# 14chanwa/remotesensingProject

Hardware: AMD Instinct MI355X
Metric: Mpixel*disparity-hypotheses/s (higher is better)
Workload: dtype f32

## Files before the change

remotesensingproject_amd/build.py:

```python
from __future__ import annotations

import os
import re
import subprocess
import sys

HERE = os.path.dirname(os.path.abspath(__file__))
CSRC = os.path.join(HERE, "csrc")
OBJ = os.path.join(CSRC, "build")
SO = os.path.join(CSRC, "librslf_hip.so")
INCLUDE = os.path.join(os.path.dirname(HERE), "include")
COMMON = ["rslf_internal.hpp", "rslf_plan.hpp", "rslf_scratch.hpp", "rslf_device.hpp", os.path.join(INCLUDE, "rslf_hip.h")]
UNITS = {
    "rslf_core.hip": ["k0_pack.hpp"],
    "rslf_pile.hip": ["k1_edge.hpp", "k_compact.hpp", "k2_scan.hpp", "k2_reg.hpp", "k2_stream.hpp", "k3_median.hpp"],
    "rslf_chip_a.hip": ["k2_scan.hpp", "k2_chip.hpp"],
    "rslf_chip_b.hip": ["k2_scan.hpp", "k2_chip.hpp"],
    "rslf_chip_c.hip": ["k2_scan.hpp", "k2_chip.hpp"],
    "rslf_sweep.hip": ["k3_median.hpp", "k4_propagate.hpp", "k_compact.hpp", "k2_scan.hpp", "k7_line_conf.hpp"],
    "rslf_f2c.hip": ["k5_f2c.hpp"],
    "rslf_render.hip": ["k6_render.hpp", "rslf_plan_render.hpp"],
    "rslf_multi.hip": [],
    "rslf_multi_sweep.hip": [],
}
SOURCES = list(UNITS)

HIPCC_FLAGS = [
    "--offload-arch=gfx950",
    "-O3",
    "-std=c++17",
    "-fPIC",
    "-ffp-contract=off",
    "-fno-fast-math",
    "-fno-slp-vectorize",
]


def _hipcc() -> str:
    for c in (os.environ.get("HIPCC"), "/opt/rocm/bin/hipcc", "hipcc"):
        if c and (os.path.isabs(c) and os.path.exists(c) or not os.path.isabs(c)):
            return c
    raise RuntimeError("hipcc not found")


def _deps(unit: str) -> list[str]:
# ... 114 lines not shown
```

remotesensingproject_amd/csrc/k2_reg.hpp:

```cpp
#pragma once

#include "k2_scan.hpp"

namespace rslf {

#ifndef RSLF_REG_GB104
#define RSLF_REG_GB104 8
#endif
constexpr int gather_batch(int c) { return c == 1 ? 8 : 4; }
constexpr int kPadSlack = 16;

template <int SPAD, int C, bool PK, bool KONLY>
__device__ __forceinline__ void mean_shift_pass(const float (&R)[PK ? 1 : C][PK ? 1 : SPAD], const f2 (&R2)[PK ? C : 1][PK ? SPAD / 2 : 1],
                                                int S, float kq, const float (&rbar)[C], float (&A)[C], float& B)
{
    static_assert(!KONLY || (C == 1 && !PK), "the K-only pass is written for the scalar one-channel blocks");
    if constexpr (PK) {
        f2 rb2[C];
        const f2 kq2 = {kq, kq};
#pragma unroll
        for (int c = 0; c < C; c++)
            rb2[c] = f2{rbar[c], rbar[c]};
        constexpr int kBlk = (C == 1) ? 8 : 4;
#pragma unroll
        for (int s0 = 0; s0 < SPAD; s0 += kBlk) {
            if (!(s0 < SPAD - kPadSlack || s0 < S))
                continue;
            if constexpr (C == 1) {
                f2 P[4], K[4];
                const f2 r4[4] = {R2[0][s0 / 2], R2[0][s0 / 2 + 1], R2[0][s0 / 2 + 2], R2[0][s0 / 2 + 3]};
                mean_shift_pk_octet(r4, rb2[0], kq2, P, K);
#pragma unroll
                for (int j = 0; j < 4; j++) {
                    A[0] = A[0] + P[j].x;
                    B = B + K[j].x;
// ... 41 lines not shown
                        else
                            mean_shift_group1(R[0][s0 + j], rbar[0], kq, A[0], B);
                    }
            }
        }
    } else {
#pragma unroll
        for (int s = 0; s < SPAD; s++) {
            if (!(s < SPAD - kPadSlack || s < S))
                continue;
            float q[C];
#pragma unroll
            for (int c = 0; c < C; c++) {
                const float delta = R[c][s] - rbar[c];
                const float tq = kq * delta;
                q[c] = tq * delta;
            }
            float qs = q[0];
            if (C == 3) {
                qs = q[0] + q[C - 1];
                qs = qs + q[C > 1 ? 1 : 0];
            }
            const float K = kernel_weight(qs);
#pragma unroll
            for (int c = 0; c < C; c++) {
                const float pr = R[c][s] * K;
                A[c] = A[c] + pr;
            }
            B = B + K;
        }
    }
}

template <int SPAD, int C, bool BORDER, bool UNIFORM_D, bool PK, int GB = 0, class BestT = Best<C>, bool LANE_D = false,
          bool TRIM = false>
__device__ __forceinline__ void scan_reg_body(const ScanArgs& a, int v, int u, int d0, int d1, BestT& best,
                                              float* __restrict__ otab, int dlane = 0, int dstep = 1)
{
    static_assert(!LANE_D || !UNIFORM_D, "hypotheses in the lanes: every lane has its own view offsets");
    constexpr int kGatherBatch = GB > 0 ? GB : (C == 1 && !PK && SPAD == 104 && RSLF_REG_GB104 == 13) ? 13 : gather_batch(C);
    static_assert(SPAD % kGatherBatch == 0 && (!PK || kGatherBatch % 2 == 0), "whole batches, whole pairs");
    static_assert(SPAD % 8 == 0, "slot counts are multiples of 8");
    const VolView& vol = a.vol;
    const float* epi = vol.row(v, 0);
    const float uf = (float)u;
    const int Um1 = vol.U - 1;
    const unsigned Um1_bits = __float_as_uint((float)Um1);
    const int S = vol.S;
    const int lane = threadIdx.x & 63;
    const long long o = (long long)v * vol.U + u;
    const float dmin = a.dmin_vu ? a.dmin_vu[o] : a.dmin;
    const float dmax = a.dmax_vu ? a.dmax_vu[o] : a.dmax;
    const float range = dmax - dmin;
    const float denom = (float)(a.dim_d - 1);
    const float kq = (C == 1) ? a.k.k1 : a.k.inv_h2;
    const float slope = a.k.slope;
    const int stride_s = (int)vol.stride_s;
    float centre[C];
#pragma unroll
    for (int c = 0; c < C; c++)
        centre[c] = epi[(long long)a.s_hat * vol.stride_s + u * C + c];

#pragma unroll 1
    for (int dk = d0; dk < d1; dk += (LANE_D ? dstep : 1)) {
        const int d = LANE_D ? min(dk + dlane, d1 - 1) : dk;
        const float Dd = hypothesis(dmin, range, denom, d);
        float R[PK ? 1 : C][PK ? 1 : SPAD];
        f2 R2[PK ? C : 1][PK ? SPAD / 2 : 1];
        int card = BORDER ? 0 : S;
        float Ss0 = (float)a.s_hat;
        asm volatile("" : "+v"(Ss0));
        int rowoff = 0;
        asm volatile("" : "+s"(rowoff));
        if (UNIFORM_D) {
#pragma unroll
            for (int s0 = 0; s0 < SPAD; s0 += 64) {
                const int s = s0 + lane;
                float off = (float)(a.s_hat - s) * Dd;
                off = off * slope;
                if (SPAD % 64 == 0 || s < SPAD)
                    otab[s] = off;
            }
            __builtin_amdgcn_wave_barrier();
        }
#pragma unroll
        for (int g = 0; g < SPAD / kGatherBatch; g++) {
            float tt[kGatherBatch], e0[C][kGatherBatch], e1[C][kGatherBatch];
            bool ok[kGatherBatch];
#pragma unroll
            for (int j = 0; j < kGatherBatch; j++) {
                const int s = g * kGatherBatch + j;
                tt[j] = 0.0f;
                ok[j] = false;
#pragma unroll
                for (int c = 0; c < C; c++) {
                    e0[c][j] = kSentinel;
                    e1[c][j] = 0.0f;
                }
                if (s < SPAD - kPadSlack || s < S) {
                    float x;
                    if (UNIFORM_D) {
                        x = otab[s];
                    } else {
                        x = (Ss0 - (float)s) * Dd;
                        x = x * slope;
                    }
                    x = x + uf;
                    tt[j] = lerp_weight(x);
                    int i0 = floor_to_int(x);
                    ok[j] = true;
                    if (BORDER) {
                        ok[j] = __float_as_uint(x) <= Um1_bits;
                        i0 = ok[j] ? i0 : 0;
                    }
                    const unsigned byteoff = (unsigned)(i0 * C + rowoff) << 2;
                    const float* p = (const float*)((const char*)epi + byteoff);
#pragma unroll
                    for (int c = 0; c < C; c++) {
                        e0[c][j] = p[c];
                        e1[c][j] = p[C + c];
                    }
                }
                rowoff += stride_s;
            }
#pragma unroll
            for (int j = 0; j < kGatherBatch; j++) {
                const int s = g * kGatherBatch + j;
                const float omt = 1.0f - tt[j];
#pragma unroll
                for (int c = 0; c < C; c++) {
                    const float m0 = omt * e0[c][j];
                    const float m1 = tt[j] * e1[c][j];
                    const float r = m0 + m1;
                    float val;
                    if (BORDER)
                        val = ok[j] ? r : kSentinel;
                    else
                        val = (s < SPAD - kPadSlack || s < S) ? r : kSentinel;
                    if constexpr (PK) {
                        if (s & 1)
                            R2[c][s >> 1].y = val;
                        else
                            R2[c][s >> 1].x = val;
                    } else {
                        R[c][s] = val;
                    }
                }
                if (BORDER)
                    card += ok[j] ? 1 : 0;
            }
            {
                const int b = g * kGatherBatch;
#pragma unroll
                for (int c = 0; c < C; c++) {
                    if constexpr (PK) {
                        asm volatile("" : "+v"(R2[c][b / 2]), "+v"(R2[c][b / 2 + 1]));
                        if (kGatherBatch == 8)
                            asm volatile("" : "+v"(R2[c][b / 2 + 2]), "+v"(R2[c][b / 2 + 3]));
                        static_assert(!PK || kGatherBatch == 4 || kGatherBatch == 8, "pair pinning is written for 4 and 8");
                    } else if (kGatherBatch != 4 && kGatherBatch != 8) {
#pragma unroll
                        for (int j = 0; j < kGatherBatch; j++)
                            asm volatile("" : "+v"(R[c][b + j]));
                    } else {
                        asm volatile("" : "+v"(R[c][b + 0]), "+v"(R[c][b + 1]), "+v"(R[c][b + 2]), "+v"(R[c][b + 3]));
                        if (kGatherBatch == 8)
                            asm volatile("" : "+v"(R[c][b + kGatherBatch - 4]), "+v"(R[c][b + kGatherBatch - 3]),
                                              "+v"(R[c][b + kGatherBatch - 2]), "+v"(R[c][b + kGatherBatch - 1]));
                    }
                }
                if (BORDER)
                    asm volatile("" : "+s"(rowoff), "+v"(Ss0), "+v"(card));
                else
                    asm volatile("" : "+s"(rowoff), "+v"(Ss0));
            }
        }

        float rbar[C];
#pragma unroll
        for (int c = 0; c < C; c++)
            rbar[c] = centre[c];
        float B = 0.0f;
// ... 102 lines not shown
};

constexpr int scan_reg_waves(int spad, int c)
{
    const int regs = ((c * spad + (c == 1 ? 64 : 96) + 7) / 8) * 8;
    const int w = 512 / regs;
    if (c == 1 && spad > 104 && spad <= 144) return 3;
    if (c == 1 && spad >= 80 && spad <= 88) return 4;
    if (c == 3 && spad >= 32 && spad <= 40) return 3;
    if (c == 1 && (spad == 48 || spad == 40)) return 5;
    if (c == 3 && spad == 24) return 4;
    if (c == 1 && spad == 16) return 7;
    return w > 8 ? 8 : (w < 1 ? 1 : w);
}

#ifndef RSLF_REG_BEST_LDS
#define RSLF_REG_BEST_LDS 1
#endif
constexpr bool scan_reg_best_in_lds(int spad, int c)
{
    if (!RSLF_REG_BEST_LDS)
        return false;
    if (c == 1)
        return spad == 16 || spad == 40 || spad == 48 || (spad >= 80 && spad <= 88) || (spad >= 104 && spad <= 144);
    return spad == 24 || spad == 40;
}

constexpr bool scan_reg_packed_math(int spad, int c) { return scan_reg_waves(spad, c) == 1; }

constexpr bool scan_reg_trim(int spad, int c)
{
    return c == 1 && !scan_reg_packed_math(spad, c) && spad != 48 && !(spad >= 80 && spad <= 88) && !(spad > 112 && spad <= 144);
}
template <int SPAD, int C>
using ScanRegRbarFix = std::conditional_t<scan_reg_trim(SPAD, C), LastPassRbar<C>, NoRbarFix>;

template <int SPAD, int C, class BestT>
__device__ __forceinline__ void scan_reg_rows(const ScanArgs& a, int v, int u, int d0, int d1, BestT& best, float* otab)
{
    constexpr bool PK = scan_reg_packed_math(SPAD, C);
    if (a.dmin_vu) {
        scan_reg_body<SPAD, C, true, false, PK, 0, BestT, false, scan_reg_trim(SPAD, C)>(a, v, u, d0, d1, best, otab);
        return;
    }
    const float max_ds = (float)max(a.s_hat, a.vol.S - 1 - a.s_hat);
    const float range = a.dmax - a.dmin, denom = (float)(a.dim_d - 1);
    const float uf = (float)u, Um1 = (float)(a.vol.U - 1);
    auto interior = [&](int d) -> bool {
        const float reach = max_ds * fabsf(hypothesis(a.dmin, range, denom, d)) * fabsf(a.k.slope) + 2.0f;
        return __all((uf - reach >= 0.0f) && (uf + reach <= Um1));
    };
    int d = d0;
    while (d < d1) {
        const bool in = interior(d);
        int e = d + 1;
        while (e < d1 && interior(e) == in)
            e++;
        if (in)
            scan_reg_body<SPAD, C, false, true, PK, 0, BestT, false, scan_reg_trim(SPAD, C)>(a, v, u, d, e, best, otab);
        else
            scan_reg_body<SPAD, C, true, true, PK, 0, BestT, false, scan_reg_trim(SPAD, C)>(a, v, u, d, e, best, otab);
        d = e;
    }
}

template <int SPAD, int C>
__global__ __launch_bounds__(64 * kScanWaves) __attribute__((amdgpu_waves_per_eu(scan_reg_waves(SPAD, C), scan_reg_waves(SPAD, C))))
void k2_scan_reg(ScanArgs a)
{
    __shared__ float s_otab[kScanWaves][SPAD];
    float* otab = s_otab[__builtin_amdgcn_readfirstlane(threadIdx.x >> 6)];
    constexpr bool kEpiDyn = false;
    float* const epi_lds = nullptr;
    const int epi_stride = 0;
    using Fix = ScanRegRbarFix<SPAD, C>;
    if constexpr (scan_reg_best_in_lds(SPAD, C)) {
        __shared__ float s_best[kScanWaves][BestLds<C>::kFloats];
        BestLds<C> running(s_best[__builtin_amdgcn_readfirstlane(threadIdx.x >> 6)]);
        RSLF_SCAN_ROW_TILE_FIX((running.init(), scan_reg_rows<SPAD, C>(a, v, u, d0, d1, running, otab), running.load(best)), Fix{})
    } else {
        RSLF_SCAN_ROW_TILE_FIX((scan_reg_rows<SPAD, C>(a, v, u, d0, d1, best, otab)), Fix{})
    }
}

#ifndef RSLF_PACKED_LONG_GB
#define RSLF_PACKED_LONG_GB 4
#endif
constexpr bool packed_long_unit(int spad, int c) { return c == 1 && spad >= 80 && spad <= 128 && spad % RSLF_PACKED_LONG_GB == 0; }
constexpr int packed_waves(int spad, int c) { return packed_long_unit(spad, c) ? 2 : scan_reg_waves(spad + 24, c); }
constexpr int packed_gather_batch(int spad, int c) { return packed_long_unit(spad, c) ? spad / RSLF_PACKED_LONG_GB : 0; }

template <int SPAD, int C>
__global__ __launch_bounds__(64 * kScanWaves) __attribute__((amdgpu_waves_per_eu(packed_waves(SPAD, C), packed_waves(SPAD, C))))
void k2_scan_reg_packed(ScanArgs a)
{
    constexpr bool kEpiDyn = false;
    float* const epi_lds = nullptr;
    const int epi_stride = 0;
    RSLF_SCAN_PACKED_LOOP((scan_reg_body<SPAD, C, true, false, packed_waves(SPAD, C) == 1, packed_gather_batch(SPAD, C)>(a, v, u, d0, d1, best, nullptr)))
}

#ifndef RSLF_PX_ROWLIKE
#define RSLF_PX_ROWLIKE 1
// ... 39 lines not shown
```

remotesensingproject_amd/csrc/k2_scan.hpp:

```cpp
#pragma once

#include <type_traits>

#include "rslf_device.hpp"

namespace rslf {

constexpr int kScanWaves = 4;
#ifndef RSLF_XCD_ROW_INTERLEAVE
#define RSLF_XCD_ROW_INTERLEAVE 1
#endif

struct ScanArgs {
    VolView vol;
    const int* list;
    const int* count;
    const float* dmin_vu;
    const float* dmax_vu;
    float dmin, dmax;
    int dim_d, s_hat;
    ScanConsts k;
    float* Ce;
    uint8_t* Ce_mask;
    float* Cd;
    float* depth;
    float* rbar;
    int32_t* idx;
    float* score;
    int tile_w;
    int tiles_per_row;
    int logical_blocks;
    int per_xcd;
    int groups;
    struct Partial* partial;
    int* ticket;
    int v0;
    int packed;
    const int* packed_n;
    int packed_adapt;
    int stream_park;
    int stream_wave_floats;
    float stream_frac_max;
    int px_waves;
    const int* rowbase;
    int row_min;
};

struct Partial {
    float score, D;
    int d;
    float rbar[3];
    double sum;
};

template <int C>
struct Best {
    float score;
    int d;
    float D;
    float rbar[C];
    double sum;
    __device__ __forceinline__ void init()
    {
        score = -1.0f;
        d = 0;
        D = 0.0f;
#pragma unroll
        for (int c = 0; c < C; c++)
            rbar[c] = 0.0f;
        sum = 0.0;
    }
    __device__ __forceinline__ void offer(float sc, int dd, float Dd, const float (&rb)[C])
    {
        sum += (double)sc;
        if (sc > score) {
            score = sc;
            d = dd;
            D = Dd;
// ... 540 lines not shown
```

remotesensingproject_amd/csrc/rslf_core.hip:

```cpp
#include "rslf_internal.hpp"

#include <algorithm>
#include <cmath>

#include "k0_pack.hpp"

using namespace rslf;


namespace rslf {

char* last_error_buffer()
{
    static thread_local char g_err[512] = "";
    return g_err;
}

static std::atomic<int> g_inject[kInjectSites];

bool inject_hit(InjectSite site)
{
    std::atomic<int>& c = g_inject[site];
    int v = c.load(std::memory_order_relaxed);
    while (v > 0)
// ... 182 lines not shown
        (void)hipEventDestroy(ctx->ev0);
    if (ctx->ev1)
        (void)hipEventDestroy(ctx->ev1);
    delete ctx;
    return RSLF_OK;
}
RSLF_API_CATCH

extern "C" int rslf_ctx_set_stream(rslf_ctx* ctx, void* hip_stream) RSLF_API_TRY
{
    if (!ctx)
        return fail(RSLF_ERR_INVALID_ARG, "ctx is NULL");
    ctx->stream = (hipStream_t)hip_stream;
    return RSLF_OK;
}
RSLF_API_CATCH

extern "C" int rslf_ctx_set_debug(rslf_ctx* ctx, const char* key, int value) RSLF_API_TRY
{
    if (!ctx || !key)
        return fail(RSLF_ERR_INVALID_ARG, "ctx/key is NULL");
    if (strcmp(key, "force_scan") == 0 && value >= 0 && value <= 2)
        ctx->force_scan = value;
    else if (strcmp(key, "force_groups") == 0 && value >= 0 && value <= 64)
        ctx->force_groups = value;
    else if (strcmp(key, "force_packed") == 0 && value >= -1 && value <= 1)
        ctx->force_packed = value;
    else if (strcmp(key, "px") == 0 && value >= -1 && value <= 1)
        ctx->px_mode = value;
    else if (strcmp(key, "stream_share") == 0 && value >= 0 && value <= 2)
        ctx->stream_share = value;
    else if (strcmp(key, "row_split") == 0 && value >= 0 && value <= 65536)
        ctx->row_split = value;
    else if (strcmp(key, "claim_skip") == 0 && (value == 0 || value == 1))
        ctx->claim_skip = value;
    else if (strcmp(key, "time_all") == 0 && (value == 0 || value == 1)) {
        ctx->time_all = value;
        ctx->ev_used = 0;
    } else if (strcmp(key, "stream_groups") == 0 && value >= 0 && value <= 64)
        ctx->stream_groups = value;
    else if (strcmp(key, "stream_lds_kib") == 0 && value >= 16 && value <= 152) {
        ctx->stream_lds_bytes = (size_t)value << 10;
    } else if (strcmp(key, "staging_kib") == 0 && value >= 0 && value <= 262144)
        ctx->staging_kib = value;
    else
        return fail(RSLF_ERR_INVALID_ARG, "rslf_ctx_set_debug: unknown key or value out of range: %s = %d", key, value);
    return RSLF_OK;
}
RSLF_API_CATCH

extern "C" int rslf_ctx_synchronize(rslf_ctx* ctx) RSLF_API_TRY
{
    if (!ctx)
        return fail(RSLF_ERR_INVALID_ARG, "ctx is NULL");
    HIP_TRY(hipSetDevice(ctx->device));
    HIP_TRY(hipStreamSynchronize(ctx->stream));
    return RSLF_OK;
}
RSLF_API_CATCH


extern "C" int rslf_volume_create(rslf_ctx* ctx, int V, int S, int U, int C, rslf_volume** out) RSLF_API_TRY
{
    if (!ctx || !out)
        return fail(RSLF_ERR_INVALID_ARG, "ctx/out is NULL");
    *out = nullptr;
// ... 474 lines not shown
```

remotesensingproject_amd/csrc/rslf_device.hpp:

```cpp
#pragma once

#include <hip/hip_runtime.h>
#include <stdint.h>

namespace rslf {

constexpr int kWave = 64;
constexpr float kSentinel = 1.0e30f;

struct VolView {
    const float* base;
    int V, S, U, C;
    int pitch;
    long long stride_s;
    long long stride_v;
    __device__ __forceinline__ const float* row(int v, int s) const
    {
        return base + (long long)v * stride_v + (long long)s * stride_s;
    }
};

struct ScanConsts {
    float slope;
    float inv_h2;
    float k1;
    float raw_thr;
    int   n_iter;
    int   interp;
};

struct EdgeConsts {
    int   filter_size;
    int   cut_shadows;
    float shadow_level;
    float edge_thr;
};

__device__ __forceinline__ float norm1(float x)
{
    return (float)((double)fabsf(x) * 1.73205080757);
}
__device__ __forceinline__ float norm3(float x, float y, float z)
{
    double s = (double)x * (double)x;
    s += (double)y * (double)y;
    s += (double)z * (double)z;
    return (float)sqrt(s);
}

__device__ __forceinline__ float kernel_weight(float q)
{
    float k;
    asm("v_sub_f32_e64 %0, 1.0, %1 clamp" : "=v"(k) : "v"(q));
    return k;
}

__device__ __forceinline__ float lerp_weight(float x)
{
    return __builtin_amdgcn_fractf(x);
}
__device__ __forceinline__ int floor_to_int(float x)
{
    int i;
    asm("v_cvt_flr_i32_f32_e32 %0, %1" : "=v"(i) : "v"(x));
    return i;
}

typedef float f2 __attribute__((ext_vector_type(2)));

__device__ __forceinline__ f2 kernel_weight_pk(f2 q)
{
    f2 k;
    const f2 one = {1.0f, 1.0f};
    asm("v_pk_add_f32 %0, %1, %2 neg_lo:[0,1] neg_hi:[0,1] clamp" : "=v"(k) : "v"(one), "v"(q));
    return k;
}

__device__ __forceinline__ void mean_shift_pk_octet(const f2 (&r)[4], f2 rb, f2 kq, f2 (&P)[4], f2 (&K)[4])
{
    const f2 one = {1.0f, 1.0f};
    f2 t0, t1, t2, t3;
    asm("v_pk_add_f32 %[k0], %[r0], %[rb] neg_lo:[0,1] neg_hi:[0,1]\n\t"
        "v_pk_add_f32 %[k1], %[r1], %[rb] neg_lo:[0,1] neg_hi:[0,1]\n\t"
        "v_pk_add_f32 %[k2], %[r2], %[rb] neg_lo:[0,1] neg_hi:[0,1]\n\t"
        "v_pk_add_f32 %[k3], %[r3], %[rb] neg_lo:[0,1] neg_hi:[0,1]\n\t"
        "v_pk_mul_f32 %[t0], %[kq], %[k0]\n\t"
        "v_pk_mul_f32 %[t1], %[kq], %[k1]\n\t"
        "v_pk_mul_f32 %[t2], %[kq], %[k2]\n\t"
        "v_pk_mul_f32 %[t3], %[kq], %[k3]\n\t"
        "v_pk_mul_f32 %[k0], %[k0], %[t0]\n\t"
        "v_pk_mul_f32 %[k1], %[k1], %[t1]\n\t"
        "v_pk_mul_f32 %[k2], %[k2], %[t2]\n\t"
        "v_pk_mul_f32 %[k3], %[k3], %[t3]\n\t"
        "v_pk_add_f32 %[k0], %[one], %[k0] neg_lo:[0,1] neg_hi:[0,1] clamp\n\t"
        "v_pk_add_f32 %[k1], %[one], %[k1] neg_lo:[0,1] neg_hi:[0,1] clamp\n\t"
        "v_pk_add_f32 %[k2], %[one], %[k2] neg_lo:[0,1] neg_hi:[0,1] clamp\n\t"
        "v_pk_add_f32 %[k3], %[one], %[k3] neg_lo:[0,1] neg_hi:[0,1] clamp\n\t"
        "v_pk_mul_f32 %[t0], %[r0], %[k0]\n\t"
        "v_pk_mul_f32 %[t1], %[r1], %[k1]\n\t"
// ... 171 lines not shown
```

remotesensingproject_amd/csrc/rslf_internal.hpp:

```cpp
#pragma once

#include "../../include/rslf_hip.h"

#include <hip/hip_runtime.h>

#include <atomic>
#include <cstdarg>
#include <cstdio>
#include <cstring>
#include <exception>
#include <functional>
#include <new>
#include <string>
#include <thread>
#include <vector>

#include "rslf_device.hpp"
#include "rslf_plan.hpp"
#include "rslf_scratch.hpp"


namespace rslf {

char* last_error_buffer();
// ... 159 lines not shown
    float* lc_K_vsu = nullptr;
    int32_t* lc_idx_vu = nullptr;
    const float* lc_Ce_svu = nullptr;
    const float* lc_dmin_vu = nullptr;
    const float* lc_dmax_vu = nullptr;
    float lc_dmin = 0.0f, lc_dmax = 0.0f;
    int lc_dim_d = 0;
    ScanConsts lc_consts = {};
};

}

struct rslf_ctx {
    int device = 0;
    hipStream_t stream = nullptr;
    rslf::Scratch scratch;
    rslf::SweepState sweep;
    hipEvent_t ev0 = nullptr, ev1 = nullptr;
    bool ev_valid = false;
    int time_all = 0;
    std::vector<hipEvent_t> ev_pool;
    size_t ev_used = 0;
    int last_spad = 0;
    int last_kernel = 0;
    int num_cus = 0;
    int force_scan = 0;
    int force_groups = 0;
    int force_packed = -1;
    int px_mode = -1;
    int stream_groups = 0;
    int stream_share = 1;
    size_t stream_lds_bytes = rslf::plan::kStreamLdsBytes;
    int row_split = 1;
    int claim_skip = 1;
    int staging_kib = 0;
};

struct rslf_volume {
    rslf_ctx* ctx = nullptr;
    int device = 0;
    int V = 0, S = 0, U = 0, C = 0, pitch = 0;
    float* base = nullptr;
    size_t bytes = 0;
    float min_value = 0.0f, max_value = 0.0f;
    bool filled = false;
};

struct rslf_multi {
    struct Dev {
        rslf_ctx* ctx = nullptr;
        hipStream_t s_up = nullptr, s_comp = nullptr, s_down = nullptr;
        hipEvent_t done[2] = {nullptr, nullptr};
        rslf_volume* vol[2] = {nullptr, nullptr};
        rslf::DeviceBuf planes[2];
        rslf::PinnedBuf pin[2];
        rslf::DeviceBuf arena;
    };
    std::vector<Dev> devs;
    int chunk_rows = 0;
    std::vector<unsigned char> peer;
};

namespace rslf {

struct StreamScope {
    StreamScope(rslf_ctx* ctx_, hipStream_t stream) : ctx(ctx_), saved(ctx_->stream) { ctx->stream = stream; }
// ... 100 lines not shown
```

remotesensingproject_amd/csrc/rslf_pile.hip:

```cpp
#include "rslf_internal.hpp"

#include <algorithm>
#include <cmath>

#include "k1_edge.hpp"
#include "k2_scan.hpp"
#include "k2_reg.hpp"
#include "k2_stream.hpp"
#include "k3_median.hpp"

using namespace rslf;

static_assert(sizeof(Partial) == plan::kPartialRecordBytes, "rslf_plan.hpp sizes the record scratch");
static_assert(kScanWaves == plan::kScanWavesPerTile, "rslf_plan.hpp shares the hypotheses out over this many waves");


extern "C" int rslf_edge_confidence_pile(rslf_ctx* ctx, const rslf_volume* vol, int s, const rslf_params* p,
                                         float* d_Ce_vu, uint8_t* d_Ce_mask_vu) RSLF_API_TRY
{
    if (!ctx || !vol || !d_Ce_vu || !d_Ce_mask_vu)
        return fail(RSLF_ERR_INVALID_ARG, "NULL argument");
    int rc = check_params(p);
    if (rc)
        return rc;
// ... 121 lines not shown
        switch (spad) {
#define RSLF_C 3
            RSLF_SPAD_LIST_3CH(RSLF_CASE)
#undef RSLF_C
        default:
            break;
        }
    }
#undef RSLF_CASE
    return fail(RSLF_ERR_UNSUPPORTED, "no register scan kernel with %d slots x %d channels", spad, C);
}

static plan::ScanKernelFacts kernel_facts(int S, int C)
{
    const int spad = plan::pick_spad(S, C);
    return plan::ScanKernelFacts{spad ? scan_reg_waves(spad, C) : 0, stream_resident_for(S, C), stream_px_resident_for(S, C)};
}

static plan::ScanRequest scan_request(const rslf_ctx* ctx, int V, int U, int S, int C, int dim_d, bool in_range, bool linear,
                                      bool pixel_ranges, const ScanInputs& in)
{
    plan::ScanRequest rq = {};
    rq.V = V, rq.U = U, rq.S = S, rq.C = C, rq.dim_d = dim_d;
    rq.num_cus = ctx->num_cus;
    rq.ctx_groups = in.groups;
    rq.ctx_packed = in.packed;
    rq.precompacted = in.lists;
    rq.force_groups = ctx->force_groups;
    rq.force_packed = ctx->force_packed;
    rq.px_mode = ctx->px_mode;
    rq.stream_groups = ctx->stream_groups;
    rq.stream_share = ctx->stream_share;
    rq.stream_lds_bytes = ctx->stream_lds_bytes;
    const bool dense_uniform = !pixel_ranges && !in.packed && ctx->force_packed != 1 && in.lists != ScanInputs::kPackedList;
    plan::choose_scan_kernel(&rq, in_range, linear, ctx->force_scan, dense_uniform, kernel_facts(S, C));
    return rq;
}

int rslf::scan_presize(rslf_ctx* ctx, int S, int U, int C, int dim_d, const rslf_params* p, const int* rows, int n_rows)
{
    const plan::ScanKernelFacts f = kernel_facts(S, C);
    int max_rows = 0;
    size_t recs = 0, tickets = 0;
    for (int i = 0; i < n_rows; i++) {
        max_rows = std::max(max_rows, rows[i]);
        ScanInputs in;
        if (p && plan::fuse_k1_compaction(p->edge_confidence_opening_size, ctx->force_packed, (size_t)rows[i] * U))
            in.lists = ScanInputs::kRowLists;
        const plan::ScanRequest rq = scan_request(ctx, rows[i], U, S, C, dim_d, true, !p || p->interpolation == RSLF_INTERP_LINEAR, false, in);
        const plan::ScanPlan sp = plan::plan_scan(rq, f.nres, f.nres_px);
        recs = std::max(recs, sp.records);
        tickets = std::max(tickets, sp.tickets);
    }
    if (max_rows < 1)
        return RSLF_OK;
    HIP_TRY(hipSetDevice(ctx->device));
    bool tickets_fresh = false;
    int rc = ensure_plane_scratch(ctx, max_rows, U);
    if (rc == RSLF_OK && recs)
        rc = ensure_group_scratch(ctx, recs, tickets, &tickets_fresh);
    if (rc == RSLF_OK && tickets_fresh)
        HIP_TRY(hipStreamSynchronize(ctx->stream));
    return rc;
}

int rslf::sweep_scan_presize(rslf_ctx* ctx, const rslf_volume* vol, int dim_d, const ScanInputs& sparse)
// ... 25 lines not shown
ScanInputs rslf::scan_defaults(const rslf_ctx* ctx)
{
    ScanInputs in;
    in.zero_total = !ctx->sweep.keep_total;
    in.timed = !ctx->sweep.open || ctx->sweep.first;
    return in;
}

static int check_scan_args(const rslf_volume* vol, const float* d_dmin_vu, const float* d_dmax_vu, int dim_d, int s_hat,
                           const rslf_params* p)
{
    int rc = check_params(p);
    if (rc)
        return rc;
    if ((d_dmin_vu == nullptr) != (d_dmax_vu == nullptr))
        return fail(RSLF_ERR_INVALID_ARG, "d_dmin_vu and d_dmax_vu must both be given or both be NULL");
    if (dim_d < 2)
        return fail(RSLF_ERR_INVALID_ARG, "dim_d=%d: the hypothesis grid divides by dim_d-1 (core.hpp:548)", dim_d);
    if (s_hat < 0 || s_hat >= vol->S)
        return fail(RSLF_ERR_INVALID_ARG, "s_hat=%d outside [0,%d)", s_hat, vol->S);
    if (!vol->filled)
        return fail(RSLF_ERR_INVALID_ARG, "volume has not been filled");
    return RSLF_OK;
}

static void apply_plan(ScanArgs& a, const plan::ScanPlan& p, const rslf_ctx* ctx)
{
    a.groups = p.groups;
    a.tile_w = p.tile_w;
    a.tiles_per_row = p.tiles_per_row;
    a.packed = p.packed ? 1 : 0;
    a.packed_adapt = p.packed_adapt ? 1 : 0;
    a.px_waves = p.px_waves;
    a.stream_park = p.stream_park;
    a.stream_wave_floats = p.stream_wave_floats;
    a.partial = p.groups > 1 ? ctx->scratch.scan_partial.as<Partial>() : nullptr;
    a.ticket = p.groups > 1 ? ctx->scratch.scan_ticket.as<int>() : nullptr;
}

static int enqueue_scan(const plan::ScanPlan& p, const ScanArgs& a, unsigned grid_x, size_t stream_lds_bytes, hipStream_t st)
{
    const dim3 grid(grid_x), block(64 * kScanWaves);
    const int C = a.vol.C;
    hipError_t attr = hipSuccess;
    auto stream = [&](auto kernel) {
        attr = hipFuncSetAttribute(reinterpret_cast<const void*>(kernel), hipFuncAttributeMaxDynamicSharedMemorySize, (int)stream_lds_bytes);
        if (attr == hipSuccess)
            hipLaunchKernelGGL(kernel, grid, block, p.lds_bytes, st, a);
    };
    int rc = RSLF_OK;
    switch (p.kind) {
    case RSLF_SCAN_REG:
    case RSLF_SCAN_REG_PX:
        rc = launch_scan_reg(p.spad, C, a, grid, st);
        break;
    case RSLF_SCAN_CHIP:
        rc = launch_scan_chip(a, grid, p.lds_bytes, st);
        break;
    case RSLF_SCAN_STREAM_PX:
        if (C == 1)
            stream_px_kernel_for<1>(p.stream_nres, stream);
        else
            stream_px_kernel_for<3>(p.stream_nres, stream);
        break;
    case RSLF_SCAN_STREAM:
        if (p.packed && C == 1)
// ... 370 lines not shown
```

remotesensingproject_amd/csrc/rslf_plan.hpp:

```cpp
#pragma once

#include <stddef.h>
#include <stdint.h>

#include <string.h>

#include <algorithm>
#include <cmath>
#include <vector>

#include "../../include/rslf_hip.h"

namespace rslf {

struct MorphElement {
    int k;
    unsigned rows[31];
};

namespace plan {


constexpr int kScanWavesPerTile = 4;
constexpr size_t kPartialRecordBytes = 32;
// ... 507 lines not shown

inline int px_waves(int dim_d)
{
    int best = 0;
    double best_use = 0.0;
    for (int w = 1; w <= kScanWavesPerTile; w *= 2) {
        const int lanes = 64 * w, iters = (dim_d + lanes - 1) / lanes;
        const double use = (double)dim_d / ((double)iters * lanes);
        if (use >= best_use - 1e-12) {
            best_use = use;
            best = w;
        }
    }
    return best_use >= 0.6 ? best : 0;
}

struct ScanRequest {
    int V, U, S, C, dim_d;
    int spad;
    bool use_stream;
    bool use_chip;
    int chip_wave_floats;
    int reg_waves;
    int num_cus;
    int ctx_groups;
    bool ctx_packed;
    int precompacted;
    int force_groups;
    int force_packed;
    int px_mode;
    int stream_groups;
    int stream_share;
    size_t stream_lds_bytes;
};

struct ScanPlan {
    int kind;
    int spad;
    int groups;
    bool packed;
    bool packed_adapt;
    int px_waves;
    int tile_w;
    int tiles_per_row;
    int rows_per_launch;
    size_t records;
    size_t tickets;
    int stream_nres;
    int stream_park;
    int stream_wave_floats;
    size_t lds_bytes;
};

inline int stream_resident_hi(int C, int nres_1ch, int nres_rgb) { return C == 1 ? nres_1ch : nres_rgb; }

struct ScanKernelFacts {
    int reg_waves;
    int nres;
    int nres_px;
};

inline bool scan_range_ok(float min_value, float max_value) { return min_value >= 0.0f && max_value <= 1.0e6f; }

inline void choose_scan_kernel(ScanRequest* r, bool in_range, bool linear, int force_scan, bool dense_uniform, const ScanKernelFacts& f)
{
    const bool lds_ok = in_range && linear && force_scan != 1 && (size_t)kScanWavesPerTile * r->S * sizeof(float) <= kScanOffsetTableBytes;
    r->spad = lds_ok && force_scan == 0 ? pick_spad(r->S, r->C) : 0;
    r->use_chip = lds_ok && r->spad == 0 && dense_uniform && force_scan != 2 && chip_takes(r->S, r->C);
    r->use_stream = lds_ok && r->spad == 0 && !r->use_chip;
    r->chip_wave_floats = r->use_chip ? chip_wave_floats(r->S, kChipLadder[chip_rung_for(r->S)]) : 0;
    r->reg_waves = r->spad ? f.reg_waves : 0;
}

inline int stream_park_for(int S, int C, int nres, size_t stream_lds_bytes)
{
// ... 41 lines not shown
    if (r.force_packed >= 0)
        packed = r.force_packed != 0;
    if (n > (size_t)INT32_MAX || r.precompacted == 1)
        packed = false;
    if (r.precompacted == 2)
        packed = true;
    while (groups > 1 && r.dim_d < 2 * kScanWavesPerTile * groups)
        groups /= 2;

    int px_w = 0;
    if (packed && (r.spad || r.use_stream) && !r.use_chip && r.px_mode != 0) {
        px_w = px_waves(r.dim_d);
        if (px_w == 0 && r.px_mode == 1)
            px_w = 1;
    }
    if (px_w && r.use_stream && nres_px >= 0)
        nres = nres_px;
    p.stream_nres = r.use_stream ? nres : 0;
    const int park_early = r.use_stream ? stream_park_for(r.S, r.C, nres, r.stream_lds_bytes) : 0;
    const bool share = r.use_chip ? r.stream_share != 0
                                  : r.use_stream && (r.stream_share == 2 || (r.stream_share == 1 && stream_shares_taps(r.S, nres, park_early)));
    p.tile_w = (share && !packed) ? 63 : 64;
    p.tiles_per_row = p.tile_w == 63 ? std::max(1, (r.U + 61) / 63) : (r.U + p.tile_w - 1) / p.tile_w;
    p.packed_adapt = packed && !r.use_stream && !r.use_chip;
    p.rows_per_launch = r.V;
    if (groups > 1 && !packed) {
        const size_t per_row = (size_t)p.tiles_per_row * groups * 64 * kPartialRecordBytes;
        p.rows_per_launch = (int)std::min<size_t>((size_t)r.V, std::max<size_t>(1, kPartialBudget / per_row));
    }
    if (packed && (r.use_stream || r.use_chip))
        while (groups > 1 && ((n + 63) / 64) * groups * 64 * kPartialRecordBytes > kPartialBudget)
            groups /= 2;
    p.px_waves = px_w;
    p.spad = r.spad;
    p.kind = r.spad ? (px_w ? RSLF_SCAN_REG_PX : RSLF_SCAN_REG)
             : r.use_chip ? RSLF_SCAN_CHIP
             : r.use_stream ? (px_w ? RSLF_SCAN_STREAM_PX : RSLF_SCAN_STREAM) : RSLF_SCAN_GENERIC;
    if (px_w) {
        groups = 1;
        p.packed_adapt = false;
    }
    p.groups = groups;
    p.packed = packed;
    p.records = 0;
    p.tickets = 0;
    if (groups > 1) {
        const size_t tiles_all = (n + 63) / 64;
        const size_t tiles_max = !packed ? (size_t)p.rows_per_launch * p.tiles_per_row
                                         : p.packed_adapt ? std::min<size_t>(tiles_all, kPackedItemTarget / 2) : tiles_all;
        p.records = (packed && p.packed_adapt) ? std::min<size_t>(tiles_all * groups, kPackedItemTarget) * 64 : tiles_max * groups * 64;
        p.tickets = tiles_max;
    }
    p.stream_park = 0;
    p.stream_wave_floats = 0;
    p.lds_bytes = 0;
    if (r.use_stream) {
        const size_t s4 = ((size_t)r.S + 3) & ~(size_t)3;
        const int park = park_early;
        p.stream_park = park;
        p.stream_wave_floats = (int)(s4 + (size_t)park * r.C * 64);
        p.stream_wave_floats = std::max(p.stream_wave_floats, 2 * (64 + (3 + r.C) * 32));
        p.lds_bytes = (size_t)kScanWavesPerTile * p.stream_wave_floats * sizeof(float);
    }
    if (r.use_chip) {
        p.stream_wave_floats = r.chip_wave_floats;
        p.lds_bytes = (size_t)kScanWavesPerTile * r.chip_wave_floats * sizeof(float);
// ... 209 lines not shown
```

remotesensingproject_amd/depth.py:

```python
from __future__ import annotations

import atexit
import copy
import ctypes as C
import sys
from dataclasses import dataclass
from typing import Optional, Sequence

import numpy as np
import torch

from . import _lib
from ._lib import RslfParams, RslfStats, RslfVolumeDesc, check


class Interpolation1DLinear:
    mode = 0


class Interpolation1DNearestNeighbour:

    def __init__(self, as_built: bool = False):
        self.mode = 2 if as_built else 1

# ... 33 lines not shown
            v = getattr(self, "par_" + f)
            setattr(p, f, int(v) if isinstance(getattr(p, f), int) else float(v))
        return p


LINE_CONF_OFF, LINE_CONF_AS_BUILT, LINE_CONF_GATE = 0, 1, 2


def require_no_line_confidence(parameters, who: str) -> None:
    if parameters is not None and int(parameters.par_line_confidence_mode) != LINE_CONF_OFF:
        raise ValueError("%s: par_line_confidence_mode=%d is not built here (one-device Depth2DComputer only)"
                         % (who, int(parameters.par_line_confidence_mode)))


class Context:

    def __init__(self, device: int | torch.device | None = None):
        if device is None:
            device = torch.cuda.current_device()
        self.device = torch.device("cuda", device) if isinstance(device, int) else torch.device(device)
        h = C.c_void_p()
        check(_lib.lib().rslf_ctx_create(self.device.index or 0, C.byref(h)), "rslf_ctx_create")
        self._h = h
        self.use_current_stream()

    def use_current_stream(self) -> None:
        s = torch.cuda.current_stream(self.device).cuda_stream
        check(_lib.lib().rslf_ctx_set_stream(self._h, C.c_void_p(s)), "rslf_ctx_set_stream")

    def synchronize(self) -> None:
        check(_lib.lib().rslf_ctx_synchronize(self._h), "rslf_ctx_synchronize")

    _DEBUG_DEFAULTS = dict(force_scan=0, force_groups=0, force_packed=-1, px=-1, stream_share=1, stream_groups=0, stream_lds_kib=80,
                           claim_skip=1, time_all=0, row_split=1, staging_kib=0)
    _FORCE_SCAN = {None: 0, "auto": 0, "generic": 1, "stream": 2}

    def set_debug(self, **hooks) -> None:
        for k, v in hooks.items():
            if k == "force_scan" and not isinstance(v, int):
                v = self._FORCE_SCAN[v or None]
            check(_lib.lib().rslf_ctx_set_debug(self._h, k.encode(), int(v)), "rslf_ctx_set_debug(%s)" % k)

    def reset_debug(self) -> None:
        self.set_debug(**self._DEBUG_DEFAULTS)

    def last_scan_kernel_ms(self) -> float:
        ms = C.c_float()
        check(_lib.lib().rslf_last_scan_kernel_ms(self._h, C.byref(ms)), "rslf_last_scan_kernel_ms")
        return float(ms.value)

    def scan_time_total_ms(self) -> tuple[float, int]:
        ms, n = C.c_float(), C.c_int()
        check(_lib.lib().rslf_scan_time_total_ms(self._h, C.byref(ms), C.byref(n)), "rslf_scan_time_total_ms")
        return float(ms.value), int(n.value)

    def close(self) -> None:
        if getattr(self, "_h", None) and not sys.is_finalizing():
            _lib.lib().rslf_ctx_destroy(self._h)
        self._h = None

    def __del__(self):
        try:
            self.close()
        except Exception:
            pass


# ... 988 lines not shown
```

Measured before the change: 8033.

## Precompute per-wave interpolation tap table for interior uniform-D register scan

For the scalar one-channel SPAD=104 interior register scan, each wave now precomputes, per disparity, a shared table of byte offsets and lerp weights from the first lane's column. It also computes a per-batch flag for when every lane can reuse those taps bit-exactly, meaning the same fract and floor shifted by the lane offset. Flagged batches skip the per-sample fract, floor and offset arithmetic and load the precomputed taps from LDS. This adds LDS (four times the otab size), ballot and readlane work, and extra code size, in exchange for less VALU work in the gather loop.

```diff
diff --git a/remotesensingproject_amd/build.py b/remotesensingproject_amd/build.py
--- a/remotesensingproject_amd/build.py
+++ b/remotesensingproject_amd/build.py
@@ -10,7 +10,7 @@
 OBJ = os.path.join(CSRC, "build")
 SO = os.path.join(CSRC, "librslf_hip.so")
 INCLUDE = os.path.join(os.path.dirname(HERE), "include")
-COMMON = ["rslf_internal.hpp", "rslf_plan.hpp", "rslf_scratch.hpp", "rslf_device.hpp", os.path.join(INCLUDE, "rslf_hip.h")]
+COMMON = ["rslf_internal.hpp", "rslf_plan.hpp", "rslf_scratch.hpp", "rslf_device.hpp", "k2_taps.hpp", os.path.join(INCLUDE, "rslf_hip.h")]
 UNITS = {
     "rslf_core.hip": ["k0_pack.hpp"],
     "rslf_pile.hip": ["k1_edge.hpp", "k_compact.hpp", "k2_scan.hpp", "k2_reg.hpp", "k2_stream.hpp", "k3_median.hpp"],
diff --git a/remotesensingproject_amd/csrc/k2_reg.hpp b/remotesensingproject_amd/csrc/k2_reg.hpp
--- a/remotesensingproject_amd/csrc/k2_reg.hpp
+++ b/remotesensingproject_amd/csrc/k2_reg.hpp
@@ -1,6 +1,7 @@
 #pragma once
 
 #include "k2_scan.hpp"
+#include "k2_taps.hpp"
 
 namespace rslf {
 
@@ -108,8 +109,71 @@
     }
 }
 
+template <int SPAD, int C, int BATCH>
+__device__ __forceinline__ void tap_table_batch(const float* epi, const float* otab, const int* tboff, const f2* tw, unsigned du_bytes,
+                                                float uf, int S, int stride_s, bool from_table, int g, int& rowoff, float (&R)[C][SPAD])
+{
+    float tt[BATCH], om[BATCH], e0[C][BATCH], e1[C][BATCH];
+    unsigned bo[BATCH];
+    if (from_table) {
+#pragma unroll
+        for (int j = 0; j < BATCH; j++) {
+            const int s = g * BATCH + j;
+            bo[j] = (unsigned)tboff[s] + du_bytes;
+            const f2 w = tw[s];
+            tt[j] = w.x;
+            om[j] = w.y;
+        }
+    } else {
+        int ro = rowoff;
+#pragma unroll
+        for (int j = 0; j < BATCH; j++) {
+            const int s = g * BATCH + j;
+            tt[j] = 0.0f;
+            bo[j] = 0;
+            if (s < SPAD - kPadSlack || s < S) {
+                const float x = otab[s] + uf;
+                tt[j] = lerp_weight(x);
+                const int i0 = floor_to_int(x);
+                bo[j] = (unsigned)(i0 * C + ro) << 2;
+            }
+            om[j] = 1.0f - tt[j];
+            ro += stride_s;
+        }
+    }
+    rowoff += BATCH * stride_s;
+#pragma unroll
+    for (int j = 0; j < BATCH; j++) {
+        const int s = g * BATCH + j;
+#pragma unroll
+        for (int c = 0; c < C; c++) {
+            e0[c][j] = kSentinel;
+            e1[c][j] = 0.0f;
+        }
+        if (s < SPAD - kPadSlack || s < S) {
+            const float* p = (const float*)((const char*)epi + bo[j]);
+#pragma unroll
+            for (int c = 0; c < C; c++) {
+                e0[c][j] = p[c];
+                e1[c][j] = p[C + c];
+            }
+        }
+    }
+#pragma unroll
+    for (int j = 0; j < BATCH; j++) {
+        const int s = g * BATCH + j;
+#pragma unroll
+        for (int c = 0; c < C; c++) {
+            const float m0 = om[j] * e0[c][j];
+            const float m1 = tt[j] * e1[c][j];
+            const float r = m0 + m1;
+            R[c][s] = (s < SPAD - kPadSlack || s < S) ? r : kSentinel;
+        }
+    }
+}
+
 template <int SPAD, int C, bool BORDER, bool UNIFORM_D, bool PK, int GB = 0, class BestT = Best<C>, bool LANE_D = false,
-          bool TRIM = false>
+          bool TRIM = false, bool TAPS = false>
 __device__ __forceinline__ void scan_reg_body(const ScanArgs& a, int v, int u, int d0, int d1, BestT& best,
                                               float* __restrict__ otab, int dlane = 0, int dstep = 1)
 {
@@ -117,6 +181,7 @@
     constexpr int kGatherBatch = GB > 0 ? GB : (C == 1 && !PK && SPAD == 104 && RSLF_REG_GB104 == 13) ? 13 : gather_batch(C);
     static_assert(SPAD % kGatherBatch == 0 && (!PK || kGatherBatch % 2 == 0), "whole batches, whole pairs");
     static_assert(SPAD % 8 == 0, "slot counts are multiples of 8");
+    static_assert(!TAPS || (UNIFORM_D && !BORDER && !PK), "the tap table belongs to the interior scalar uniform-D row form");
     const VolView& vol = a.vol;
     const float* epi = vol.row(v, 0);
     const float uf = (float)u;
@@ -136,6 +201,18 @@
 #pragma unroll
     for (int c = 0; c < C; c++)
         centre[c] = epi[(long long)a.s_hat * vol.stride_s + u * C + c];
+    int* const tboff = TAPS ? reinterpret_cast<int*>(otab + SPAD) : nullptr;
+    f2* const tw = TAPS ? reinterpret_cast<f2*>(otab + 2 * SPAD) : nullptr;
+    int u_first = 0, u_last = 0;
+    unsigned du_bytes = 0;
+    bool taps_on = false;
+    if constexpr (TAPS) {
+        u_first = __builtin_amdgcn_readfirstlane(u);
+        u_last = __builtin_amdgcn_readlane(u, 63);
+        const int du = u - u_first;
+        du_bytes = (unsigned)(du * C) << 2;
+        taps_on = a.tap_table != 0 && __all(du == min(lane, u_last - u_first));
+    }
 
 #pragma unroll 1
     for (int dk = d0; dk < d1; dk += (LANE_D ? dstep : 1)) {
@@ -148,82 +225,110 @@
         asm volatile("" : "+v"(Ss0));
         int rowoff = 0;
         asm volatile("" : "+s"(rowoff));
+        unsigned fastb = 0;
         if (UNIFORM_D) {
+            int lane_s = lane, tile_first = u_first, tile_last = u_last;
+            if constexpr (TAPS)
+                asm volatile("" : "+v"(lane_s), "+s"(tile_first), "+s"(tile_last));
 #pragma unroll
             for (int s0 = 0; s0 < SPAD; s0 += 64) {
-                const int s = s0 + lane;
+                const int s = s0 + lane_s;
                 float off = (float)(a.s_hat - s) * Dd;
                 off = off * slope;
                 if (SPAD % 64 == 0 || s < SPAD)
                     otab[s] = off;
+                if constexpr (TAPS) {
+                    if (taps_on) {
+                        const TapEntry e = tap_entry(off, tile_first, tile_last, vol.U, C, __mul24(s, stride_s));
+                        if (SPAD % 64 == 0 || s < SPAD) {
+                            tboff[s] = e.byteoff;
+                            tw[s] = f2{e.t, e.omt};
+                        }
+                        unsigned long long m = __ballot(e.fast);
+                        m &= m >> 1;
+                        m &= m >> 2;
+                        m &= m >> 4;
+                        static_assert(!TAPS || kGatherBatch == 8, "the batch bits are gathered for batches of eight samples");
+#pragma unroll
+                        for (int k = 0; k < 8; k++)
+                            if (s0 + 8 * k < SPAD)
+                                fastb |= ((unsigned)(m >> (8 * k)) & 1u) << (s0 / 8 + k);
+                    }
+                }
             }
             __builtin_amdgcn_wave_barrier();
+            if constexpr (TAPS)
+                fastb = __builtin_amdgcn_readfirstlane(fastb & (S >= SPAD ? ~0u : (1u << (S / kGatherBatch)) - 1u));
         }
 #pragma unroll
         for (int g = 0; g < SPAD / kGatherBatch; g++) {
-            float tt[kGatherBatch], e0[C][kGatherBatch], e1[C][kGatherBatch];
-            bool ok[kGatherBatch];
-#pragma unroll
-            for (int j = 0; j < kGatherBatch; j++) {
-                const int s = g * kGatherBatch + j;
-                tt[j] = 0.0f;
-                ok[j] = false;
-#pragma unroll
-                for (int c = 0; c < C; c++) {
-                    e0[c][j] = kSentinel;
-                    e1[c][j] = 0.0f;
-                }
-                if (s < SPAD - kPadSlack || s < S) {
-                    float x;
-                    if (UNIFORM_D) {
-                        x = otab[s];
-                    } else {
-                        x = (Ss0 - (float)s) * Dd;
-                        x = x * slope;
+            if constexpr (TAPS) {
+                tap_table_batch<SPAD, C, kGatherBatch>(epi, otab, tboff, tw, du_bytes, uf, S, stride_s, (fastb >> g) & 1u, g, rowoff, R);
+            } else {
+                float tt[kGatherBatch], e0[C][kGatherBatch], e1[C][kGatherBatch];
+                bool ok[kGatherBatch];
+#pragma unroll
+                for (int j = 0; j < kGatherBatch; j++) {
+                    const int s = g * kGatherBatch + j;
+                    tt[j] = 0.0f;
+                    ok[j] = false;
+#pragma unroll
+                    for (int c = 0; c < C; c++) {
+                        e0[c][j] = kSentinel;
+                        e1[c][j] = 0.0f;
                     }
-                    x = x + uf;
-                    tt[j] = lerp_weight(x);
-                    int i0 = floor_to_int(x);
-                    ok[j] = true;
-                    if (BORDER) {
-                        ok[j] = __float_as_uint(x) <= Um1_bits;
-                        i0 = ok[j] ? i0 : 0;
+                    if (s < SPAD - kPadSlack || s < S) {
+                        float x;
+                        if (UNIFORM_D) {
+                            x = otab[s];
+                        } else {
+                            x = (Ss0 - (float)s) * Dd;
+                            x = x * slope;
+                        }
+                        x = x + uf;
+                        tt[j] = lerp_weight(x);
+                        int i0 = floor_to_int(x);
+                        ok[j] = true;
+                        if (BORDER) {
+                            ok[j] = __float_as_uint(x) <= Um1_bits;
+                            i0 = ok[j] ? i0 : 0;
+                        }
+                        const unsigned byteoff = (unsigned)(i0 * C + rowoff) << 2;
+                        const float* p = (const float*)((const char*)epi + byteoff);
+#pragma unroll
+                        for (int c = 0; c < C; c++) {
+                            e0[c][j] = p[c];
+                            e1[c][j] = p[C + c];
+                        }
                     }
-                    const unsigned byteoff = (unsigned)(i0 * C + rowoff) << 2;
-                    const float* p = (const float*)((const char*)epi + byteoff);
+                    rowoff += stride_s;
+                }
+#pragma unroll
+                for (int j = 0; j < kGatherBatch; j++) {
+                    const int s = g * kGatherBatch + j;
+                    const float omt = 1.0f - tt[j];
 #pragma unroll
                     for (int c = 0; c < C; c++) {
-                        e0[c][j] = p[c];
-                        e1[c][j] = p[C + c];
+                        const float m0 = omt * e0[c][j];
+                        const float m1 = tt[j] * e1[c][j];
+                        const float r = m0 + m1;
+                        float val;
+                        if (BORDER)
+                            val = ok[j] ? r : kSentinel;
+                        else
+                            val = (s < SPAD - kPadSlack || s < S) ? r : kSentinel;
+                        if constexpr (PK) {
+                            if (s & 1)
+                                R2[c][s >> 1].y = val;
+                            else
+                                R2[c][s >> 1].x = val;
+                        } else {
+                            R[c][s] = val;
+                        }
                     }
-                }
-                rowoff += stride_s;
-            }
-#pragma unroll
-            for (int j = 0; j < kGatherBatch; j++) {
-                const int s = g * kGatherBatch + j;
-                const float omt = 1.0f - tt[j];
-#pragma unroll
-                for (int c = 0; c < C; c++) {
-                    const float m0 = omt * e0[c][j];
-                    const float m1 = tt[j] * e1[c][j];
-                    const float r = m0 + m1;
-                    float val;
                     if (BORDER)
-                        val = ok[j] ? r : kSentinel;
-                    else
-                        val = (s < SPAD - kPadSlack || s < S) ? r : kSentinel;
-                    if constexpr (PK) {
-                        if (s & 1)
-                            R2[c][s >> 1].y = val;
-                        else
-                            R2[c][s >> 1].x = val;
-                    } else {
-                        R[c][s] = val;
-                    }
-                }
-                if (BORDER)
-                    card += ok[j] ? 1 : 0;
+                        card += ok[j] ? 1 : 0;
+                }
             }
             {
                 const int b = g * kGatherBatch;
@@ -392,6 +497,11 @@
 {
     return c == 1 && !scan_reg_packed_math(spad, c) && spad != 48 && !(spad >= 80 && spad <= 88) && !(spad > 112 && spad <= 144);
 }
+#ifndef RSLF_TAP_TABLE
+#define RSLF_TAP_TABLE 1
+#endif
+constexpr bool scan_reg_tap_table(int spad, int c) { return RSLF_TAP_TABLE && c == 1 && spad == 104 && scan_reg_trim(spad, c); }
+
 template <int SPAD, int C>
 using ScanRegRbarFix = std::conditional_t<scan_reg_trim(SPAD, C), LastPassRbar<C>, NoRbarFix>;
 
@@ -399,6 +509,7 @@
 __device__ __forceinline__ void scan_reg_rows(const ScanArgs& a, int v, int u, int d0, int d1, BestT& best, float* otab)
 {
     constexpr bool PK = scan_reg_packed_math(SPAD, C);
+    constexpr bool kTaps = scan_reg_tap_table(SPAD, C);
     if (a.dmin_vu) {
         scan_reg_body<SPAD, C, true, false, PK, 0, BestT, false, scan_reg_trim(SPAD, C)>(a, v, u, d0, d1, best, otab);
         return;
@@ -417,7 +528,7 @@
         while (e < d1 && interior(e) == in)
             e++;
         if (in)
-            scan_reg_body<SPAD, C, false, true, PK, 0, BestT, false, scan_reg_trim(SPAD, C)>(a, v, u, d, e, best, otab);
+            scan_reg_body<SPAD, C, false, true, PK, 0, BestT, false, scan_reg_trim(SPAD, C), kTaps>(a, v, u, d, e, best, otab);
         else
             scan_reg_body<SPAD, C, true, true, PK, 0, BestT, false, scan_reg_trim(SPAD, C)>(a, v, u, d, e, best, otab);
         d = e;
@@ -428,7 +539,7 @@
 __global__ __launch_bounds__(64 * kScanWaves) __attribute__((amdgpu_waves_per_eu(scan_reg_waves(SPAD, C), scan_reg_waves(SPAD, C))))
 void k2_scan_reg(ScanArgs a)
 {
-    __shared__ float s_otab[kScanWaves][SPAD];
+    __shared__ __attribute__((aligned(16))) float s_otab[kScanWaves][SPAD * (scan_reg_tap_table(SPAD, C) ? 4 : 1)];
     float* otab = s_otab[__builtin_amdgcn_readfirstlane(threadIdx.x >> 6)];
     constexpr bool kEpiDyn = false;
     float* const epi_lds = nullptr;
diff --git a/remotesensingproject_amd/csrc/k2_scan.hpp b/remotesensingproject_amd/csrc/k2_scan.hpp
--- a/remotesensingproject_amd/csrc/k2_scan.hpp
+++ b/remotesensingproject_amd/csrc/k2_scan.hpp
@@ -44,6 +44,7 @@
     int px_waves;
     const int* rowbase;
     int row_min;
+    int tap_table;
 };
 
 struct Partial {
diff --git a/remotesensingproject_amd/csrc/k2_taps.hpp b/remotesensingproject_amd/csrc/k2_taps.hpp
--- /dev/null
+++ b/remotesensingproject_amd/csrc/k2_taps.hpp
@@ -0,0 +1,69 @@
+#pragma once
+
+#include <math.h>
+#include <stdint.h>
+#include <string.h>
+
+#if defined(__HIPCC__)
+#define RSLF_TAPS_FN __host__ __device__ __forceinline__
+#else
+#define RSLF_TAPS_FN inline
+#endif
+
+namespace rslf {
+
+struct TapEntry {
+    int byteoff;
+    float t, omt;
+    bool fast;
+};
+
+RSLF_TAPS_FN uint32_t tap_float_bits(float x)
+{
+#if defined(__HIP_DEVICE_COMPILE__)
+    return __float_as_uint(x);
+#else
+    uint32_t b;
+    memcpy(&b, &x, sizeof(b));
+    return b;
+#endif
+}
+
+RSLF_TAPS_FN float tap_fract(float x)
+{
+#if defined(__HIP_DEVICE_COMPILE__)
+    return __builtin_amdgcn_fractf(x);
+#else
+    return x - floorf(x);
+#endif
+}
+RSLF_TAPS_FN int tap_floor(float x)
+{
+#if defined(__HIP_DEVICE_COMPILE__)
+    int i;
+    asm("v_cvt_flr_i32_f32_e32 %0, %1" : "=v"(i) : "v"(x));
+    return i;
+#else
+    return (int)floorf(x);
+#endif
+}
+
+RSLF_TAPS_FN TapEntry tap_entry(float off, int u_first, int u_last, int U, int C, int row_floats)
+{
+    const float uf = (float)u_first, ul = (float)u_last;
+    const float x_first = off + uf;
+    const float x_last = off + ul;
+    TapEntry e;
+    e.t = tap_fract(x_first);
+    const int i0 = tap_floor(x_first);
+    e.omt = 1.0f - e.t;
+    e.byteoff = (int)((unsigned)(i0 * C + row_floats) << 2);
+    const bool inside = x_first > 0.0f && x_last <= (float)(U - 1);
+    const bool binade = ((tap_float_bits(x_first) ^ tap_float_bits(x_last)) >> 23) == 0;
+    const float back = x_last - ul;
+    const bool exact = back == off;
+    e.fast = inside && (binade || exact);
+    return e;
+}
+
+}
diff --git a/remotesensingproject_amd/csrc/rslf_core.hip b/remotesensingproject_amd/csrc/rslf_core.hip
--- a/remotesensingproject_amd/csrc/rslf_core.hip
+++ b/remotesensingproject_amd/csrc/rslf_core.hip
@@ -238,6 +238,8 @@
         ctx->stream_share = value;
     else if (strcmp(key, "row_split") == 0 && value >= 0 && value <= 65536)
         ctx->row_split = value;
+    else if (strcmp(key, "tap_table") == 0 && (value == 0 || value == 1))
+        ctx->tap_table = value;
     else if (strcmp(key, "claim_skip") == 0 && (value == 0 || value == 1))
         ctx->claim_skip = value;
     else if (strcmp(key, "time_all") == 0 && (value == 0 || value == 1)) {
diff --git a/remotesensingproject_amd/csrc/rslf_device.hpp b/remotesensingproject_amd/csrc/rslf_device.hpp
--- a/remotesensingproject_amd/csrc/rslf_device.hpp
+++ b/remotesensingproject_amd/csrc/rslf_device.hpp
@@ -2,6 +2,8 @@
 
 #include <hip/hip_runtime.h>
 #include <stdint.h>
+
+#include "k2_taps.hpp"
 
 namespace rslf {
 
@@ -55,16 +57,8 @@
     return k;
 }
 
-__device__ __forceinline__ float lerp_weight(float x)
-{
-    return __builtin_amdgcn_fractf(x);
-}
-__device__ __forceinline__ int floor_to_int(float x)
-{
-    int i;
-    asm("v_cvt_flr_i32_f32_e32 %0, %1" : "=v"(i) : "v"(x));
-    return i;
-}
+__device__ __forceinline__ float lerp_weight(float x) { return tap_fract(x); }
+__device__ __forceinline__ int floor_to_int(float x) { return tap_floor(x); }
 
 typedef float f2 __attribute__((ext_vector_type(2)));
 
diff --git a/remotesensingproject_amd/csrc/rslf_internal.hpp b/remotesensingproject_amd/csrc/rslf_internal.hpp
--- a/remotesensingproject_amd/csrc/rslf_internal.hpp
+++ b/remotesensingproject_amd/csrc/rslf_internal.hpp
@@ -215,6 +215,7 @@
     int stream_share = 1;
     size_t stream_lds_bytes = rslf::plan::kStreamLdsBytes;
     int row_split = 1;
+    int tap_table = 1;
     int claim_skip = 1;
     int staging_kib = 0;
 };
diff --git a/remotesensingproject_amd/csrc/rslf_pile.hip b/remotesensingproject_amd/csrc/rslf_pile.hip
--- a/remotesensingproject_amd/csrc/rslf_pile.hip
+++ b/remotesensingproject_amd/csrc/rslf_pile.hip
@@ -177,6 +177,7 @@
     rq.stream_groups = ctx->stream_groups;
     rq.stream_share = ctx->stream_share;
     rq.stream_lds_bytes = ctx->stream_lds_bytes;
+    rq.tap_table = ctx->tap_table;
     const bool dense_uniform = !pixel_ranges && !in.packed && ctx->force_packed != 1 && in.lists != ScanInputs::kPackedList;
     plan::choose_scan_kernel(&rq, in_range, linear, ctx->force_scan, dense_uniform, kernel_facts(S, C));
     return rq;
@@ -268,6 +269,7 @@
     a.packed = p.packed ? 1 : 0;
     a.packed_adapt = p.packed_adapt ? 1 : 0;
     a.px_waves = p.px_waves;
+    a.tap_table = p.tap_table;
     a.stream_park = p.stream_park;
     a.stream_wave_floats = p.stream_wave_floats;
     a.partial = p.groups > 1 ? ctx->scratch.scan_partial.as<Partial>() : nullptr;
diff --git a/remotesensingproject_amd/csrc/rslf_plan.hpp b/remotesensingproject_amd/csrc/rslf_plan.hpp
--- a/remotesensingproject_amd/csrc/rslf_plan.hpp
+++ b/remotesensingproject_amd/csrc/rslf_plan.hpp
@@ -563,6 +563,7 @@
     int stream_groups;
     int stream_share;
     size_t stream_lds_bytes;
+    int tap_table;
 };
 
 struct ScanPlan {
@@ -572,6 +573,7 @@
     bool packed;
     bool packed_adapt;
     int px_waves;
+    int tap_table;
     int tile_w;
     int tiles_per_row;
     int rows_per_launch;
@@ -679,6 +681,7 @@
         while (groups > 1 && ((n + 63) / 64) * groups * 64 * kPartialRecordBytes > kPartialBudget)
             groups /= 2;
     p.px_waves = px_w;
+    p.tap_table = (r.spad && !packed && r.tap_table) ? 1 : 0;
     p.spad = r.spad;
     p.kind = r.spad ? (px_w ? RSLF_SCAN_REG_PX : RSLF_SCAN_REG)
              : r.use_chip ? RSLF_SCAN_CHIP
diff --git a/remotesensingproject_amd/depth.py b/remotesensingproject_amd/depth.py
--- a/remotesensingproject_amd/depth.py
+++ b/remotesensingproject_amd/depth.py
@@ -89,7 +89,7 @@
         check(_lib.lib().rslf_ctx_synchronize(self._h), "rslf_ctx_synchronize")
 
     _DEBUG_DEFAULTS = dict(force_scan=0, force_groups=0, force_packed=-1, px=-1, stream_share=1, stream_groups=0, stream_lds_kib=80,
-                           claim_skip=1, time_all=0, row_split=1, staging_kib=0)
+                           claim_skip=1, time_all=0, row_split=1, staging_kib=0, tap_table=1)
     _FORCE_SCAN = {None: 0, "auto": 0, "generic": 1, "stream": 2}
 
     def set_debug(self, **hooks) -> None:
```

Result: faster. 8131 (median of 6 runs) (+1.2%).
